# suvajit-patra/sl-hwgat

Hardware: AMD Instinct MI355X
Metric: clips/sec fwd+bwd at B=64 T=128 J=67; %HBM roofline; 1->8 GPU scaling (higher is better)
Workload: dtype f32

## Files before the change

### sl-hwgat_amd/csrc/gemm_f32_nt256.hip

```cpp
#include <type_traits>
#include "common.h"
#include "fused_ops.h"
#include "gemm_f32.h"

namespace {

constexpr int BT = 256, BK = 32, LDT = 36;
constexpr int BUF = 2 * BT * LDT;
constexpr int SLD = 132;

constexpr int SG_MFMA = 0x008, SG_VALU = 0x002, SG_VMEM_RD = 0x020, SG_DS_RD = 0x100, SG_DS_WR = 0x200;

template <int G, int M1, int N1, int M2 = 0, int N2 = 0, int NV = 0>
__device__ __forceinline__ void pin() {
#pragma unroll
    for (int q = 0; q < G; ++q) {
        __builtin_amdgcn_sched_group_barrier(SG_MFMA, 64 / G, 0);
        if constexpr (NV > 0) __builtin_amdgcn_sched_group_barrier(SG_VALU, NV, 0);
        if constexpr (N1 > 0) __builtin_amdgcn_sched_group_barrier(M1, N1, 0);
        if constexpr (N2 > 0) __builtin_amdgcn_sched_group_barrier(M2, N2, 0);
    }
}

#ifdef HWGAT_LAB
__device__ unsigned long long* g_nt256_stamps = nullptr;
#define NT256_STAMP(i) do { if (g_nt256_stamps && threadIdx.x == 0) g_nt256_stamps[blockIdx.x * 2 + (i)] = __builtin_amdgcn_s_memtime(); } while (0)
#else
#define NT256_STAMP(i) do {} while (0)
#endif

template <int PRO, int EPI, int STAT = 0>
__global__ __launch_bounds__(256, 1) void gemm_nt256_k(NtArgs p) {
    HWGAT_RESOLVE_SEEDS2(p);
    __shared__ __attribute__((aligned(16))) float sm[2 * BUF];
    const int tid = threadIdx.x, lane = tid & 63, wave = tid >> 6;
    const int lq = lane & 31, hh = lane >> 5;
    const int wm = wave >> 1, wn = wave & 1;
    const int tiles_n = p.N / BT;
    const int row_blocks = (int)(p.M / BT);
    const int n_tiles = row_blocks * tiles_n;
    const int n_slab = p.K / BK;
    const int lrow = tid >> 3, lc4 = (tid & 7) * 4;
    const uint32_t pro_th = drop_thresh(p.pro_p);
    const float pro_sc = 1.0f / (1.0f - p.pro_p);

    f32x4 ra[8], rw[8];
    float ln_mean[8], ln_rstd[8];
    f32x4 ln_g, ln_b;

    const int swz_tiles = (row_blocks / 8) * 8 * tiles_n;
    auto tile_origin = [&](int t, int64_t& m0, int& n0) {
        int rb, nt;
        if (t < swz_tiles) {
            rb = (t / (8 * tiles_n)) * 8 + (t & 7);
            nt = (t >> 3) % tiles_n;
        } else {
            const int w = t - swz_tiles;
            rb = (row_blocks / 8) * 8 + w / tiles_n;
            nt = w % tiles_n;
        }
        m0 = (int64_t)rb * BT;
        n0 = nt * BT;
    };
    const float* pa; const float* pw;
    auto set_tile = [&](int64_t m0, int n0) {
        pa = p.A + (m0 + lrow) * p.K + lc4;
        pw = p.W + (int64_t)(n0 + lrow) * p.K + lc4;
        if constexpr (PRO == PRO_LN) {
#pragma unroll
            for (int i = 0; i < 8; ++i) { ln_mean[i] = p.mean[m0 + lrow + 32 * i]; ln_rstd[i] = p.rstd[m0 + lrow + 32 * i]; }
        }
    };
    const int64_t rstep = (int64_t)32 * p.K;
    auto issue = [&](int slab) {
        const float* a = pa + slab * BK;
        const float* w = pw + slab * BK;
#pragma unroll
        for (int i = 0; i < 8; ++i) {
            ra[i] = *reinterpret_cast<const f32x4*>(a + i * rstep);
            rw[i] = *reinterpret_cast<const f32x4*>(w + i * rstep);
        }
        if constexpr (PRO == PRO_LN) {
            ln_g = *reinterpret_cast<const f32x4*>(p.gamma + slab * BK + lc4);
            ln_b = *reinterpret_cast<const f32x4*>(p.beta + slab * BK + lc4);
        }
    };
    auto commit = [&](int buf, int64_t m0, int slab) {
        float* As = sm + buf * BUF + lrow * LDT + lc4;
        float* Ws = As + BT * LDT;
#pragma unroll
        for (int i = 0; i < 8; ++i) {
            f32x4 a = ra[i];
            if constexpr (PRO == PRO_LN) {
                a = (a - ln_mean[i]) * (ln_rstd[i] * ln_g) + ln_b;
            } else if constexpr (PRO == PRO_DROP) {
                a *= drop_keep4(p.pro_seed, (uint64_t)(m0 + lrow + 32 * i) * p.K + slab * BK + lc4, pro_th, pro_sc);
            }
            *reinterpret_cast<f32x4*>(As + i * 32 * LDT) = a;
            *reinterpret_cast<f32x4*>(Ws + i * 32 * LDT) = rw[i];
        }
    };
    constexpr int PRO_VALU = PRO == PRO_LN ? 14 : (PRO == PRO_DROP ? 44 : 0);

    f32x16 acc[4][4];
    struct Frag { f32x4 a[4], b[4]; };
    Frag f0, f1;
    auto fetch = [&](Frag& f, int buf, int kk) {
        const float* ap = sm + buf * BUF + (wm * 128 + lq) * LDT + 4 * hh + 8 * kk;
        const float* wp = sm + buf * BUF + BT * LDT + (wn * 128 + lq) * LDT + 4 * hh + 8 * kk;
#pragma unroll
        for (int i = 0; i < 4; ++i) {
            f.a[i] = *reinterpret_cast<const f32x4*>(ap + i * 32 * LDT);
            f.b[i] = *reinterpret_cast<const f32x4*>(wp + i * 32 * LDT);
        }
    };
    auto mfma64 = [&](const Frag& f) {
#pragma unroll
        for (int e = 0; e < 4; ++e)
#pragma unroll
            for (int i = 0; i < 4; ++i)
#pragma unroll
                for (int j = 0; j < 4; ++j)
                    acc[i][j] = __builtin_amdgcn_mfma_f32_32x32x2f32(f.a[i][e], f.b[j][e], acc[i][j], 0, 0, 0);
    };
    auto slab_body = [&](int buf, int64_t m_next, int s_next) {
        fetch(f1, buf, 1);
        issue(s_next);
        mfma64(f0);
        pin<16, SG_DS_RD, 1, SG_VMEM_RD, 1>();
        __builtin_amdgcn_sched_barrier(0);
        fetch(f0, buf, 2);
        mfma64(f1);
        pin<8, SG_DS_RD, 1>();
        __builtin_amdgcn_sched_barrier(0);
        fetch(f1, buf, 3);
        commit(buf ^ 1, m_next, s_next);
        mfma64(f0);
        pin<8, SG_DS_WR, 2, SG_DS_RD, 1, PRO_VALU>();
        __builtin_amdgcn_sched_barrier(0);
        mfma64(f1);
        __builtin_amdgcn_sched_barrier(0);
        __syncthreads();
    };

    int t = blockIdx.x;
    if (t >= n_tiles) return;
    int64_t m0; int n0;
    tile_origin(t, m0, n0);
    set_tile(m0, n0);
    NT256_STAMP(0);
    issue(0);
    commit(0, m0, 0);
    __syncthreads();
    int buf = 0;

    while (true) {
#pragma unroll
        for (int i = 0; i < 4; ++i)
#pragma unroll
            for (int j = 0; j < 4; ++j)
#pragma unroll
                for (int e = 0; e < 16; ++e) acc[i][j][e] = 0.f;

        const int tn = t + gridDim.x;
        int64_t mn = m0; int nn = n0;
        for (int s = 0; s < n_slab; ++s) {
            const bool last = s + 1 == n_slab;
            if (last) {
                if (tn < n_tiles) tile_origin(tn, mn, nn);
                set_tile(mn, nn);
            }
            fetch(f0, buf, 0);
            slab_body(buf, last ? mn : m0, last ? 0 : s + 1);
            buf ^= 1;
        }

        {
            const uint32_t epi_th = drop_thresh(p.epi_p);
            const float epi_sc = 1.0f / (1.0f - p.epi_p);
            float* stg = sm + (buf ^ 1) * BUF + wave * (32 * SLD);
            const int er = lane >> 5, ec = (lane & 31) * 4;
            float* rowstat = sm + (buf ^ 1) * BUF + 4 * (32 * SLD);
            static_assert(STAT == X_NONE || STAT == X_LNFOLD || 4 * 32 * SLD + 4 * BT <= BUF, "no room for the row statistics");
            const int col = n0 + wn * 128 + ec;
            f32x4 bv = {0.f, 0.f, 0.f, 0.f};
            if constexpr (epi_has_bias(EPI))
                if (p.bias) bv = *reinterpret_cast<const f32x4*>(p.bias + col);
            f32x4 sv = bv, cv = bv;
            if constexpr (STAT == X_LNFOLD) {
                sv = *reinterpret_cast<const f32x4*>(p.gamma + col);
                cv = *reinterpret_cast<const f32x4*>(p.beta + col);
            }
#pragma unroll
            for (int i = 0; i < 4; ++i) {
                const int64_t off0 = (m0 + wm * 128 + i * 32 + er) * p.N + col;
                float rr[16], rm[16];
                if constexpr (STAT == X_LNFOLD) {
                    const int64_t r0 = m0 + wm * 128 + i * 32 + er;
#pragma unroll
                    for (int ps = 0; ps < 16; ++ps) { rr[ps] = p.rstd[r0 + 2 * ps]; rm[ps] = p.mean[r0 + 2 * ps]; }
                }
                const int64_t rs2 = 2 * (int64_t)p.N;
                MergeWalk mw;
                if constexpr (STAT == X_STAT_MERGE) mw.start(m0 + wm * 128 + i * 32 + er, p.mg_F, p.mg_K, 2);
                f32x4 ex[16];
                if constexpr (epi_reads_extra(EPI)) {
                    const float* src = (EPI == EPI_BIAS_DROP_RES ? p.res : p.aux) + off0;
#pragma unroll
                    for (int ps = 0; ps < 16; ++ps) ex[ps] = *reinterpret_cast<const f32x4*>(src + ps * rs2);
                }
#pragma unroll
                for (int j = 0; j < 4; ++j)
#pragma unroll
                    for (int r = 0; r < 16; ++r) stg[crow(r, hh) * SLD + j * 32 + lq] = acc[i][j][r];
                __builtin_amdgcn_fence(__ATOMIC_ACQ_REL, "wavefront");
                __builtin_amdgcn_wave_barrier();
#pragma unroll
                for (int ps = 0; ps < 16; ++ps) {
                    const int64_t off = off0 + ps * rs2;
                    f32x4 v = *reinterpret_cast<const f32x4*>(stg + (2 * ps + er) * SLD + ec);
                    if constexpr (STAT == X_LNFOLD) v = v * rr[ps] + (cv - sv * (rm[ps] * rr[ps]));
                    else v += bv;
                    f32x4 dk = {1.f, 1.f, 1.f, 1.f};
                    if constexpr (epi_drops(EPI)) {
                        dk = drop_keep4(p.epi_seed, (uint64_t)off, epi_th, epi_sc);
                    }
                    if constexpr (EPI == EPI_BIAS_DROP_RES) {
                        v = ex[ps] + v * dk;
                    } else if constexpr (EPI == EPI_BIAS_GELU_DROP) {
                        *reinterpret_cast<f32x4*>(p.C2 + off) = v;
                        v.x = gelu_f(v.x) * dk.x; v.y = gelu_f(v.y) * dk.y;
                        v.z = gelu_f(v.z) * dk.z; v.w = gelu_f(v.w) * dk.w;
                    } else if constexpr (EPI == EPI_BIAS_GELU_DROP_G) {
                        float u4[4] = {v.x, v.y, v.z, v.w}, g4[4];
                        const float k4[4] = {dk.x, dk.y, dk.z, dk.w};
#pragma unroll
                        for (int e = 0; e < 4; ++e) gelu_fwd_grad(u4[e], k4[e], u4[e], g4[e]);
                        v = f32x4{u4[0], u4[1], u4[2], u4[3]};
                        const f32x4 gq = {g4[0], g4[1], g4[2], g4[3]};
                        *reinterpret_cast<f32x4*>(p.C2 + off) = gq;
                    } else if constexpr (EPI == EPI_MUL_AUX) {
                        v *= ex[ps];
                    } else if constexpr (EPI == EPI_GELU_BWD) {
                        const f32x4 h = ex[ps];
                        v.x *= dk.x * gelu_grad(h.x); v.y *= dk.y * gelu_grad(h.y);
                        v.z *= dk.z * gelu_grad(h.z); v.w *= dk.w * gelu_grad(h.w);
                    }
                    if constexpr (STAT == X_STAT || STAT == X_STAT_MERGE) {
                        float s1 = (v.x + v.y) + (v.z + v.w), s2 = (v.x * v.x + v.y * v.y) + (v.z * v.z + v.w * v.w);
                        s1 = group_sum<32>(s1); s2 = group_sum<32>(s2);
                        const int lr = wm * 128 + i * 32 + 2 * ps + er;
                        if ((lane & 31) == 0) { f32x2 st = {s1, s2}; *reinterpret_cast<f32x2*>(rowstat + (wn * BT + lr) * 2) = st; }
                        if constexpr (STAT == X_STAT_MERGE) {
                            *reinterpret_cast<f32x4*>(p.C + mw.off(p.N) + col) = v;
                            mw.next();
                        } else {
                            *reinterpret_cast<f32x4*>(p.C + off) = v;
                        }
                    } else {
                        *reinterpret_cast<f32x4*>(p.C + off) = v;
                    }
                }
                __builtin_amdgcn_fence(__ATOMIC_ACQ_REL, "wavefront");
                __builtin_amdgcn_wave_barrier();
            }
            if constexpr (STAT == X_STAT || STAT == X_STAT_MERGE) {
                __syncthreads();
                int64_t mr = m0 + tid;
                if constexpr (STAT == X_STAT_MERGE) { MergeWalk w; w.start(m0 + tid, p.mg_F, p.mg_K, 1); mr = w.mrow(); }
                atomicAdd(p.stat_sum + mr, rowstat[2 * tid] + rowstat[2 * (BT + tid)]);
                atomicAdd(p.stat_sq + mr, rowstat[2 * tid + 1] + rowstat[2 * (BT + tid) + 1]);
            }
        }
        __syncthreads();
        t = tn;
        if (t >= n_tiles) break;
        m0 = mn; n0 = nn;
    }
    NT256_STAMP(1);
}

template <int PRO>
int launch(const NtArgs& a, int epi, int grid, hipStream_t st, bool fold = false) {
    if (a.stat_sum != nullptr) {
        if constexpr (PRO == PRO_NONE) {
            if (a.mg_K > 0) gemm_nt256_k<PRO_NONE, EPI_BIAS_DROP_RES, 2><<<grid, 256, 0, st>>>(a);
            else gemm_nt256_k<PRO_NONE, EPI_BIAS_DROP_RES, 1><<<grid, 256, 0, st>>>(a);
            HWGAT_LAUNCH_CHECK();
        }
        return HWGAT_EINVAL;
    }
    if (fold) {
        if constexpr (PRO == PRO_NONE) {
            if (epi == EPI_BIAS) gemm_nt256_k<PRO_NONE, EPI_BIAS, X_LNFOLD><<<grid, 256, 0, st>>>(a);
            else if (epi == EPI_BIAS_GELU_DROP) gemm_nt256_k<PRO_NONE, EPI_BIAS_GELU_DROP, X_LNFOLD><<<grid, 256, 0, st>>>(a);
            else if (epi == EPI_BIAS_GELU_DROP_G) gemm_nt256_k<PRO_NONE, EPI_BIAS_GELU_DROP_G, X_LNFOLD><<<grid, 256, 0, st>>>(a);
            else return HWGAT_EINVAL;
            HWGAT_LAUNCH_CHECK();
        }
        return HWGAT_EINVAL;
    }
    switch (epi) {
        case EPI_BIAS: gemm_nt256_k<PRO, EPI_BIAS><<<grid, 256, 0, st>>>(a); break;
        case EPI_BIAS_DROP_RES: gemm_nt256_k<PRO, EPI_BIAS_DROP_RES><<<grid, 256, 0, st>>>(a); break;
        case EPI_BIAS_GELU_DROP: gemm_nt256_k<PRO, EPI_BIAS_GELU_DROP><<<grid, 256, 0, st>>>(a); break;
        case EPI_GELU_BWD: gemm_nt256_k<PRO, EPI_GELU_BWD><<<grid, 256, 0, st>>>(a); break;
        case EPI_BIAS_GELU_DROP_G: gemm_nt256_k<PRO, EPI_BIAS_GELU_DROP_G><<<grid, 256, 0, st>>>(a); break;
        case EPI_MUL_AUX: gemm_nt256_k<PRO, EPI_MUL_AUX><<<grid, 256, 0, st>>>(a); break;
        case EPI_NONE: gemm_nt256_k<PRO, EPI_NONE><<<grid, 256, 0, st>>>(a); break;
        default: return HWGAT_EINVAL;
    }
    HWGAT_LAUNCH_CHECK();
}

}

int hwgat_launch_nt256(const NtArgs& a, int pro, int epi, hipStream_t st) {
    if (a.M % BT || a.N % BT || a.K % BK) return HWGAT_ESHAPE;
    const int64_t tiles = (a.M / BT) * (a.N / BT);
    if (tiles > 0x7fffffff) return HWGAT_ESHAPE;
    const int grid = (int)(tiles < 256 ? tiles : 256);
    switch (pro) {
        case PRO_NONE: return launch<PRO_NONE>(a, epi, grid, st);
        case PRO_LN_FOLD: return launch<PRO_NONE>(a, epi, grid, st, true);
        case PRO_LN: return launch<PRO_LN>(a, epi, grid, st);
        case PRO_DROP: return launch<PRO_DROP>(a, epi, grid, st);
        default: return HWGAT_EINVAL;
    }
}

#ifdef HWGAT_LAB
extern "C" int hwgat_lab_nt256_stamps(void* buf) {
    return hipMemcpyToSymbol(HIP_SYMBOL(g_nt256_stamps), &buf, sizeof(buf)) == hipSuccess ? 0 : HWGAT_EINVAL;
}
#endif
```

Baseline: 640.4.

## Overlap next-tile slab prefetch and extra-operand loads with GEMM epilogue

During the epilogue of a persistent tile, the kernel now issues the global loads for the next tile's second K-slab and commits them after the epilogue, so the first slab iteration of the next tile skips its own staging. Residual/aux extra operands are double-buffered in chunks of 8 or 16 rows and requested ahead of use instead of all 16 at once per row block. LN-fold row statistics are loaded once per wave into LDS rather than 32 scalar loads per block. The aim is to hide global-load latency in the epilogue and cut register pressure, at the cost of more complex buffer-reuse logic and an LDS region that now must always fit (static_assert tightened).

```diff
diff --git a/sl-hwgat_amd/csrc/gemm_f32_nt256.hip b/sl-hwgat_amd/csrc/gemm_f32_nt256.hip
--- a/sl-hwgat_amd/csrc/gemm_f32_nt256.hip
+++ b/sl-hwgat_amd/csrc/gemm_f32_nt256.hip
@@ -123,9 +123,9 @@
                 for (int j = 0; j < 4; ++j)
                     acc[i][j] = __builtin_amdgcn_mfma_f32_32x32x2f32(f.a[i][e], f.b[j][e], acc[i][j], 0, 0, 0);
     };
-    auto slab_body = [&](int buf, int64_t m_next, int s_next) {
+    auto slab_body = [&](int buf, int64_t m_next, int s_next, bool stage) {
         fetch(f1, buf, 1);
-        issue(s_next);
+        if (stage) issue(s_next);
         mfma64(f0);
         pin<16, SG_DS_RD, 1, SG_VMEM_RD, 1>();
         __builtin_amdgcn_sched_barrier(0);
@@ -134,7 +134,7 @@
         pin<8, SG_DS_RD, 1>();
         __builtin_amdgcn_sched_barrier(0);
         fetch(f1, buf, 3);
-        commit(buf ^ 1, m_next, s_next);
+        if (stage) commit(buf ^ 1, m_next, s_next);
         mfma64(f0);
         pin<8, SG_DS_WR, 2, SG_DS_RD, 1, PRO_VALU>();
         __builtin_amdgcn_sched_barrier(0);
@@ -153,6 +153,8 @@
     commit(0, m0, 0);
     __syncthreads();
     int buf = 0;
+    bool pre = false;
+    const int s_pre = n_slab >= 2 ? 1 : 0;
 
     while (true) {
 #pragma unroll
@@ -171,7 +173,7 @@
                 set_tile(mn, nn);
             }
             fetch(f0, buf, 0);
-            slab_body(buf, last ? mn : m0, last ? 0 : s + 1);
+            slab_body(buf, last ? mn : m0, last ? 0 : s + 1, !(pre && s == 0));
             buf ^= 1;
         }
 
@@ -181,7 +183,7 @@
             float* stg = sm + (buf ^ 1) * BUF + wave * (32 * SLD);
             const int er = lane >> 5, ec = (lane & 31) * 4;
             float* rowstat = sm + (buf ^ 1) * BUF + 4 * (32 * SLD);
-            static_assert(STAT == X_NONE || STAT == X_LNFOLD || 4 * 32 * SLD + 4 * BT <= BUF, "no room for the row statistics");
+            static_assert(4 * 32 * SLD + 4 * BT <= BUF, "no room for the row statistics");
             const int col = n0 + wn * 128 + ec;
             f32x4 bv = {0.f, 0.f, 0.f, 0.f};
             if constexpr (epi_has_bias(EPI))
@@ -191,24 +193,35 @@
                 sv = *reinterpret_cast<const f32x4*>(p.gamma + col);
                 cv = *reinterpret_cast<const f32x4*>(p.beta + col);
             }
+            float* lnst = rowstat + wave * 256;
+            float lnv[4];
+            if constexpr (STAT == X_LNFOLD) {
+                const int64_t r0 = m0 + wm * 128 + lane;
+                lnv[0] = p.rstd[r0]; lnv[1] = p.rstd[r0 + 64]; lnv[2] = p.mean[r0]; lnv[3] = p.mean[r0 + 64];
+            }
+            const int64_t rs2 = 2 * (int64_t)p.N;
+            constexpr int EXN = (PRO == PRO_LN || (PRO == PRO_DROP && EPI == EPI_GELU_BWD)) ? 8 : 16, NS = 64 / EXN;
+            f32x4 exa[EXN], exb[EXN];
+            auto request = [&](f32x4 (&ex)[EXN], int k) {
+                if constexpr (epi_reads_extra(EPI)) {
+                    const float* src = (EPI == EPI_BIAS_DROP_RES ? p.res : p.aux) + (m0 + wm * 128 + 2 * k * EXN + er) * p.N + col;
+#pragma unroll
+                    for (int q = 0; q < EXN; ++q) ex[q] = *reinterpret_cast<const f32x4*>(src + q * rs2);
+                }
+            };
+            request(exa, 0);
+            __builtin_amdgcn_sched_barrier(0);
+            issue(s_pre);
+            __builtin_amdgcn_sched_barrier(0);
+            if constexpr (STAT == X_LNFOLD) {
+                lnst[lane] = lnv[0]; lnst[64 + lane] = lnv[1]; lnst[128 + lane] = lnv[2]; lnst[192 + lane] = lnv[3];
+            }
 #pragma unroll
             for (int i = 0; i < 4; ++i) {
                 const int64_t off0 = (m0 + wm * 128 + i * 32 + er) * p.N + col;
-                float rr[16], rm[16];
-                if constexpr (STAT == X_LNFOLD) {
-                    const int64_t r0 = m0 + wm * 128 + i * 32 + er;
-#pragma unroll
-                    for (int ps = 0; ps < 16; ++ps) { rr[ps] = p.rstd[r0 + 2 * ps]; rm[ps] = p.mean[r0 + 2 * ps]; }
-                }
-                const int64_t rs2 = 2 * (int64_t)p.N;
                 MergeWalk mw;
                 if constexpr (STAT == X_STAT_MERGE) mw.start(m0 + wm * 128 + i * 32 + er, p.mg_F, p.mg_K, 2);
-                f32x4 ex[16];
-                if constexpr (epi_reads_extra(EPI)) {
-                    const float* src = (EPI == EPI_BIAS_DROP_RES ? p.res : p.aux) + off0;
-#pragma unroll
-                    for (int ps = 0; ps < 16; ++ps) ex[ps] = *reinterpret_cast<const f32x4*>(src + ps * rs2);
-                }
+                if (i * 16 / EXN + 1 < NS) request(((i * 16 / EXN) & 1) ? exa : exb, i * 16 / EXN + 1);
 #pragma unroll
                 for (int j = 0; j < 4; ++j)
 #pragma unroll
@@ -218,15 +231,20 @@
 #pragma unroll
                 for (int ps = 0; ps < 16; ++ps) {
                     const int64_t off = off0 + ps * rs2;
+                    const int k = (i * 16 + ps) / EXN;
+                    if (ps > 0 && ps % EXN == 0 && k + 1 < NS) request((k & 1) ? exa : exb, k + 1);
+                    const f32x4& exv = ((k & 1) ? exb : exa)[ps % EXN];
                     f32x4 v = *reinterpret_cast<const f32x4*>(stg + (2 * ps + er) * SLD + ec);
-                    if constexpr (STAT == X_LNFOLD) v = v * rr[ps] + (cv - sv * (rm[ps] * rr[ps]));
-                    else v += bv;
+                    if constexpr (STAT == X_LNFOLD) {
+                        const float rr = lnst[i * 32 + 2 * ps + er], rm = lnst[128 + i * 32 + 2 * ps + er];
+                        v = v * rr + (cv - sv * (rm * rr));
+                    } else v += bv;
                     f32x4 dk = {1.f, 1.f, 1.f, 1.f};
                     if constexpr (epi_drops(EPI)) {
                         dk = drop_keep4(p.epi_seed, (uint64_t)off, epi_th, epi_sc);
                     }
                     if constexpr (EPI == EPI_BIAS_DROP_RES) {
-                        v = ex[ps] + v * dk;
+                        v = exv + v * dk;
                     } else if constexpr (EPI == EPI_BIAS_GELU_DROP) {
                         *reinterpret_cast<f32x4*>(p.C2 + off) = v;
                         v.x = gelu_f(v.x) * dk.x; v.y = gelu_f(v.y) * dk.y;
@@ -240,9 +258,9 @@
                         const f32x4 gq = {g4[0], g4[1], g4[2], g4[3]};
                         *reinterpret_cast<f32x4*>(p.C2 + off) = gq;
                     } else if constexpr (EPI == EPI_MUL_AUX) {
-                        v *= ex[ps];
+                        v *= exv;
                     } else if constexpr (EPI == EPI_GELU_BWD) {
-                        const f32x4 h = ex[ps];
+                        const f32x4 h = exv;
                         v.x *= dk.x * gelu_grad(h.x); v.y *= dk.y * gelu_grad(h.y);
                         v.z *= dk.z * gelu_grad(h.z); v.w *= dk.w * gelu_grad(h.w);
                     }
@@ -276,6 +294,8 @@
         t = tn;
         if (t >= n_tiles) break;
         m0 = mn; n0 = nn;
+        pre = n_slab >= 2;
+        if (pre) commit(buf ^ 1, m0, 1);
     }
     NT256_STAMP(1);
 }
```

New measurement: 636.6. No clear change (-0.6%).
